# CAMMA-public/SelfPose3d

Hardware: AMD Instinct MI355X
Metric: multi-view samples/sec (5-view Panoptic, 80x80x20 voxel) (higher is better)
Workload: dtype f32

## Files before the change

### selfpose3d_amd/csrc/sp3d_winograd.hip

```cpp
#include <hip/hip_runtime.h>
#include <stdint.h>

#include "../../include/sp3d.h"

namespace sp3d {

__device__ __forceinline__ void bt4(float &d0, float &d1, float &d2, float &d3)
{
    const float t0 = d0 - d2, t1 = d1 + d2, t2 = d2 - d1, t3 = d1 - d3;
    d0 = t0; d1 = t1; d2 = t2; d3 = t3;
}

__global__ __launch_bounds__(256) void wino_input_kernel(const float *__restrict__ x, float *__restrict__ V, int B, int X,
                                                        int Y, int Z, int C, int TX, int TY, int TZ)
{
    const int64_t T = (int64_t)B * TX * TY * TZ;
    const int64_t gid = (int64_t)blockIdx.x * 256 + threadIdx.x;
    if (gid >= T * C) return;
    const int c = (int)(gid % C);
    int64_t t = gid / C;
    const int tz = (int)(t % TZ); int64_t r = t / TZ;
    const int ty = (int)(r % TY); r /= TY;
    const int tx = (int)(r % TX);
    const int b = (int)(r / TX);
// ... 407 lines not shown
            (void)r;
            w.mh = u32x4{0x3f803f80u + (unsigned)jk, 0x3f803f80u, 0x3f803f80u + (unsigned)i, 0x3f803f80u};
            w.l = u32x2{0x3f803f80u, 0x3f803f80u};
#else
            w.mh = *reinterpret_cast<const u32x4_a8 *>(r);
            w.l = *reinterpret_cast<const u32x2_a8 *>(r + 4);
#endif
            return w;
        };
        auto step = [&](int jk, int jk_next, const WfB (&bcur)[2], WfB (&bnxt)[2]) {
            const int j = jk >> 2, k = jk & 3;
            const int ya = (j == 0) ? 0 : ((j == 2) ? 2 : 1), yb = (j == 3) ? 3 : ((j == 2) ? 1 : 2);
            const int za = (k == 0) ? 0 : ((k == 2) ? 2 : 1), zb = (k == 3) ? 3 : ((k == 2) ? 1 : 2);
            const float sy = (j == 1) ? 1.0f : -1.0f, sz = (k == 1) ? 1.0f : -1.0f;
            const float *r00 = rb + (za * WF_RY + ya) * WF_ROW, *r10 = rb + (za * WF_RY + yb) * WF_ROW;
            const float *r01 = rb + (zb * WF_RY + ya) * WF_ROW, *r11 = rb + (zb * WF_RY + yb) * WF_ROW;
            WfB blate[2];
            blate[0] = load_b(2, jk);
            blate[1] = load_b(3, jk);
            float g[4][4];
#pragma unroll
            for (int xi = 0; xi < 4; ++xi) {
#if SP3D_W16_ABLATE & 8
                const float f0 = __int_as_float(0x3f800000 + jk + xi), f1 = __int_as_float(0x3f900000 + lane);
                const float4 v00 = make_float4(f0, f1, f0, f1), v10 = make_float4(f1, f0, f1, f0), v01 = v00, v11 = v10;
                (void)r00; (void)r10; (void)r01; (void)r11;
#else
                const float4 v00 = *reinterpret_cast<const float4 *>(r00 + xi * WF_VS), v10 = *reinterpret_cast<const float4 *>(r10 + xi * WF_VS);
                const float4 v01 = *reinterpret_cast<const float4 *>(r01 + xi * WF_VS), v11 = *reinterpret_cast<const float4 *>(r11 + xi * WF_VS);
#endif
                g[xi][0] = fmaf(sz, fmaf(sy, v11.x, v01.x), fmaf(sy, v10.x, v00.x));
                g[xi][1] = fmaf(sz, fmaf(sy, v11.y, v01.y), fmaf(sy, v10.y, v00.y));
                g[xi][2] = fmaf(sz, fmaf(sy, v11.z, v01.z), fmaf(sy, v10.z, v00.z));
                g[xi][3] = fmaf(sz, fmaf(sy, v11.w, v01.w), fmaf(sy, v10.w, v00.w));
            }
            float cyz[4];
#pragma unroll
            for (int bc = 0; bc < 4; ++bc) {
                const int bb = bc >> 1, c2 = bc & 1;
                const float cy = bb == 0 ? (j < 3 ? 1.0f : 0.0f) : (j == 0 ? 0.0f : (j == 1 ? 1.0f : -1.0f));
                const float cz = c2 == 0 ? (k < 3 ? 1.0f : 0.0f) : (k == 0 ? 0.0f : (k == 1 ? 1.0f : -1.0f));
                cyz[bc] = cy * cz;
            }
            f32x16 M0, M1;
#pragma unroll
            for (int v = 0; v < 16; ++v) { M0[v] = 0.0f; M1[v] = 0.0f; }
#pragma unroll
            for (int i = 0; i < 4; ++i) {
                float av[4];
#pragma unroll
                for (int kk = 0; kk < 4; ++kk)
                    av[kk] = (i == 1) ? g[1][kk] + g[2][kk] : ((i == 3) ? g[3][kk] - g[1][kk] : g[wf_ta(i)][kk] - g[wf_tb(i)][kk]);
                const unsigned hi01 = pack_bf16(av[0], av[1]), hi23 = pack_bf16(av[2], av[3]);
#if SP3D_W16_ABLATE & 4
                const unsigned mid01 = hi01, mid23 = hi23, lo01 = hi01, lo23 = hi23;
#else
                const float r0 = av[0] - bf16_lo(hi01), r1 = av[1] - bf16_hi(hi01), r2 = av[2] - bf16_lo(hi23), r3 = av[3] - bf16_hi(hi23);
                const unsigned mid01 = pack_bf16(r0, r1), mid23 = pack_bf16(r2, r3);
                const unsigned lo01 = pack_bf16(r0 - bf16_lo(mid01), r1 - bf16_hi(mid01));
                const unsigned lo23 = pack_bf16(r2 - bf16_lo(mid23), r3 - bf16_hi(mid23));
#endif
                const u32x4 Qhh = {hi01, hi23, hi01, hi23}, Qmm = {mid01, mid23, mid01, mid23}, Qlh = {lo01, lo23, hi01, hi23};
                const WfB &w = (i < 2) ? bcur[i] : blate[i - 2];
                const u32x4 Bmh = w.mh;
                const u32x4 Bhl = {w.mh.z, w.mh.w, w.l.x, w.l.y};
#if SP3D_W16_ABLATE & 1
                {
                    const unsigned z = (Qhh.x ^ Bmh.x) + (Qmm.y ^ Bmh.z) + (Qlh.x ^ Bhl.w) + (Qlh.z ^ Bhl.y);
                    M0[0] += __uint_as_float(z & 0x3fffffffu);
                    M1[1] += __uint_as_float((z >> 1) & 0x3fffffffu);
                    if (i == 1) {
                        bnxt[0] = load_b(0, jk_next);
                        bnxt[1] = load_b(1, jk_next);
                    }
                    continue;
                }
#endif
                if (i < 3) {
                    M0 = mfma_bf16(Qhh, Bmh, M0);
                    M0 = mfma_bf16(Qmm, Bmh, M0);
                    M0 = mfma_bf16(Qlh, Bhl, M0);
                }
                if (i == 1 || i == 3) {
                    M1 = mfma_bf16(Qhh, Bmh, M1);
                    M1 = mfma_bf16(Qmm, Bmh, M1);
                    M1 = mfma_bf16(Qlh, Bhl, M1);
                }
                if (i == 2) {
                    const u32x4 nmh = Bmh ^ 0x80008000u, nhl = Bhl ^ 0x80008000u;
                    M1 = mfma_bf16(Qhh, nmh, M1);
                    M1 = mfma_bf16(Qmm, nmh, M1);
                    M1 = mfma_bf16(Qlh, nhl, M1);
                }
                if (i == 1) {
                    bnxt[0] = load_b(0, jk_next);
                    bnxt[1] = load_b(1, jk_next);
                }
            }
#pragma unroll
            for (int bc = 0; bc < 4; ++bc) {
                const float coef = cyz[bc];
                if (coef != 0.0f) {
                    f32x16 cv;
#pragma unroll
                    for (int v = 0; v < 16; ++v) cv[v] = coef;
                    acc[bc] = __builtin_elementwise_fma(M0, cv, acc[bc]);
                    acc[4 + bc] = __builtin_elementwise_fma(M1, cv, acc[4 + bc]);
                }
            }
        };
        WfB b0[2], b1[2];
        b0[0] = load_b(0, 0);
        b0[1] = load_b(1, 0);
#pragma unroll 1
        for (int jk = 0; jk < 16; jk += 2) {
            step(jk, jk + 1, b0, b1);
            step(jk + 1, (jk + 2) & 15, b1, b0);
        }
    }

    const float sh = shift[t];
    const int yl = oy0 + 2 * h;
    const int64_t obase = ((((int64_t)b * X + ox0) * Y + yl) * Z + oz0) * O + t;
#pragma unroll
    for (int a = 0; a < 8; ++a) {
        float rv[16];
        if (MODE >= 2) {
#pragma unroll
            for (int v = 0; v < 16; ++v) {
                const int dx = 2 * (v & 3) + (a >> 2), dy = 4 * ((v >> 2) & 1) + ((a >> 1) & 1), dz = 2 * (v >> 3) + (a & 1);
                const int xo = min(ox0 + dx, X - 1), yo = min(yl + dy, Y - 1), zo = min(oz0 + dz, Z - 1);
                rv[v] = res[((((int64_t)b * X + xo) * Y + yo) * Z + zo) * O + t];
            }
        }
#pragma unroll
        for (int v = 0; v < 16; ++v) {
            const int dx = 2 * (v & 3) + (a >> 2), dy = 4 * ((v >> 2) & 1) + ((a >> 1) & 1), dz = 2 * (v >> 3) + (a & 1);
            if (ox0 + dx < X && oz0 + dz < Z && yl + dy < Y) {
                const int64_t idx = obase + (((int64_t)dx * Y + dy) * Z + dz) * O;
                float val = acc[a][v] + sh;
                if (MODE == 2) val += rv[v];
                if (MODE >= 1) val = fmaxf(val, 0.0f);
                if (MODE == 3) val += rv[v];
                y[idx] = val;
            }
        }
    }
}

typedef float f32x4 __attribute__((ext_vector_type(4)));
constexpr int W16_RX = 10, W16_RY = 10, W16_RZ = 4, W16_VS = 16;
constexpr int W16_ROW = W16_RX * W16_VS + 4;
constexpr int W16_LDS = W16_RY * W16_RZ * W16_ROW;

__device__ __forceinline__ f32x4 mfma16_bf16(u32x4 a, u32x4 b, f32x4 c)
{
    return __builtin_amdgcn_mfma_f32_16x16x32_bf16(__builtin_bit_cast(bf16x8, a), __builtin_bit_cast(bf16x8, b), c, 0, 0, 0);
}

template <int C, int MODE, int NBW, int KS>
__global__ __launch_bounds__(64 * (4 / NBW) * KS) __attribute__((amdgpu_waves_per_eu(NBW <= 2 ? 2 : 1))) void wino_fused16_kernel(const float *__restrict__ x,
                                                                          const unsigned *__restrict__ U3,
                                                                          float *__restrict__ y, const float *__restrict__ shift,
                                                                          const float *__restrict__ res, int B, int X, int Y,
                                                                          int Z, int NBX, int NBY, int NBZ)
{
    constexpr int O = 64, NCH = C / 16, NOW = 4 / NBW, NTG = 64 * NOW;
    static_assert(NCH % KS == 0, "chunks must divide evenly over the channel groups");
    __shared__ __attribute__((aligned(16))) float lds[KS * W16_LDS];
    const int tid = threadIdx.x, lane = tid & 63, wave = tid >> 6;
    const int kg = wave / NOW, ow = wave % NOW, tg = tid - kg * NTG;
    float *region = lds + kg * W16_LDS;
    const int tl = lane & 15, q = lane >> 4;
    int bid = blockIdx.x;
    const int bz = bid % NBZ; bid /= NBZ;
    const int by = bid % NBY; bid /= NBY;
    const int bx = bid % NBX;
    const int b = bid / NBX;
    const int ttx = tl & 3, tty = tl >> 2;
    const int ox0 = bx * 8, oy0 = by * 8, oz0 = bz * 2;
    const float *rb = region + (2 * tty) * W16_ROW + (2 * ttx) * W16_VS + 4 * q;

    f32x4 acc[8][NBW];
#pragma unroll
    for (int a = 0; a < 8; ++a)
#pragma unroll
        for (int n = 0; n < NBW; ++n) acc[a][n] = f32x4{0.0f, 0.0f, 0.0f, 0.0f};
#ifdef SP3D_W16_SETPRIO
    __builtin_amdgcn_s_setprio(SP3D_W16_SETPRIO);
#endif

    constexpr int NV4 = W16_RX * W16_RY * W16_RZ * 4, PER = (NV4 + NTG - 1) / NTG;
    int goff[PER], loff[PER];
#pragma unroll
    for (int u = 0; u < PER; ++u) {
        const int idx = tg + u * NTG;
        const int v = idx >> 2, part = idx & 3;
        const int vx = v % W16_RX, vy = (v / W16_RX) % W16_RY, vz = v / (W16_RX * W16_RY);
        const int gx = ox0 - 1 + vx, gy = oy0 - 1 + vy, gz = oz0 - 1 + vz;
        const bool in = idx < NV4 && gx >= 0 && gx < X && gy >= 0 && gy < Y && gz >= 0 && gz < Z;
        goff[u] = in ? (int)(((((int64_t)gx) * Y + gy) * Z + gz) * C + part * 4) : -1;
        loff[u] = idx < NV4 ? (vz * W16_RY + vy) * W16_ROW + vx * W16_VS + part * 4 : -1;
    }
    const float *xb = x + (int64_t)b * X * Y * Z * C;
    float4 pre[PER];
    auto fetch = [&](int cc) {
#pragma unroll
        for (int u = 0; u < PER; ++u) {
            pre[u] = make_float4(0.0f, 0.0f, 0.0f, 0.0f);
            if (goff[u] >= 0) pre[u] = *reinterpret_cast<const float4 *>(xb + goff[u] + cc * 16);
        }
    };
    fetch(kg);
#pragma unroll 1
    for (int cc = kg; cc < NCH; cc += KS) {
        __syncthreads();
#pragma unroll
        for (int u = 0; u < PER; ++u)
            if (loff[u] >= 0) *reinterpret_cast<float4 *>(region + loff[u]) = pre[u];
        __syncthreads();
        if (cc + KS < NCH) fetch(cc + KS);
        const unsigned *ub = U3 + ((((int64_t)cc * 4 + q) * O) + ow * NBW * 16 + tl) * 6;
        auto load_b = [&](int i, int jk, int n) {
            const unsigned *r = ub + (int64_t)(i * 16 + jk) * NCH * 4 * O * 6 + n * 16 * 6;
            WfB w;
            w.mh = *reinterpret_cast<const u32x4_a8 *>(r);
            w.l = *reinterpret_cast<const u32x2_a8 *>(r + 4);
            return w;
        };
#pragma unroll 1
        for (int jk = 0; jk < 16; ++jk) {
            const int j = jk >> 2, k = jk & 3;
            WfB bw[NBW][4];
#pragma unroll
            for (int n = 0; n < NBW; ++n)
#pragma unroll
                for (int i = 0; i < 4; ++i) {
#if SP3D_W16_ABLATE & 2
                    bw[n][i].mh = u32x4{0x3f803f80u + (unsigned)(jk + n), 0x3f803f80u, 0x3f803f80u + (unsigned)i, 0x3f803f80u};
                    bw[n][i].l = u32x2{0x3f803f80u, 0x3f803f80u};
#else
                    bw[n][i] = load_b(i, jk, n);
#endif
                }
            const int ya = (j == 0) ? 0 : ((j == 2) ? 2 : 1), yb = (j == 3) ? 3 : ((j == 2) ? 1 : 2);
            const int za = (k == 0) ? 0 : ((k == 2) ? 2 : 1), zb = (k == 3) ? 3 : ((k == 2) ? 1 : 2);
            const float sy = (j == 1) ? 1.0f : -1.0f, sz = (k == 1) ? 1.0f : -1.0f;
            const float *r00 = rb + (za * W16_RY + ya) * W16_ROW, *r10 = rb + (za * W16_RY + yb) * W16_ROW;
            const float *r01 = rb + (zb * W16_RY + ya) * W16_ROW, *r11 = rb + (zb * W16_RY + yb) * W16_ROW;
            float g[4][4];
#pragma unroll
            for (int xi = 0; xi < 4; ++xi) {
#if SP3D_W16_ABLATE & 8
                const float f0 = __int_as_float(0x3f800000 + jk + xi), f1 = __int_as_float(0x3f900000 + lane);
                const float4 v00 = make_float4(f0, f1, f0, f1), v10 = make_float4(f1, f0, f1, f0), v01 = v00, v11 = v10;
                (void)r00; (void)r10; (void)r01; (void)r11;
#else
                const float4 v00 = *reinterpret_cast<const float4 *>(r00 + xi * W16_VS), v10 = *reinterpret_cast<const float4 *>(r10 + xi * W16_VS);
                const float4 v01 = *reinterpret_cast<const float4 *>(r01 + xi * W16_VS), v11 = *reinterpret_cast<const float4 *>(r11 + xi * W16_VS);
#endif
                g[xi][0] = fmaf(sz, fmaf(sy, v11.x, v01.x), fmaf(sy, v10.x, v00.x));
                g[xi][1] = fmaf(sz, fmaf(sy, v11.y, v01.y), fmaf(sy, v10.y, v00.y));
                g[xi][2] = fmaf(sz, fmaf(sy, v11.z, v01.z), fmaf(sy, v10.z, v00.z));
                g[xi][3] = fmaf(sz, fmaf(sy, v11.w, v01.w), fmaf(sy, v10.w, v00.w));
            }
            float cyz[4];
#pragma unroll
            for (int bc = 0; bc < 4; ++bc) {
                const int bb = bc >> 1, c2 = bc & 1;
                const float cy = bb == 0 ? (j < 3 ? 1.0f : 0.0f) : (j == 0 ? 0.0f : (j == 1 ? 1.0f : -1.0f));
                const float cz = c2 == 0 ? (k < 3 ? 1.0f : 0.0f) : (k == 0 ? 0.0f : (k == 1 ? 1.0f : -1.0f));
                cyz[bc] = cy * cz;
            }
            f32x4 M0[NBW], M1[NBW];
#pragma unroll
            for (int n = 0; n < NBW; ++n) { M0[n] = f32x4{0.0f, 0.0f, 0.0f, 0.0f}; M1[n] = f32x4{0.0f, 0.0f, 0.0f, 0.0f}; }
#pragma unroll
            for (int i = 0; i < 4; ++i) {
                float av[4];
#pragma unroll
                for (int kk = 0; kk < 4; ++kk)
                    av[kk] = (i == 1) ? g[1][kk] + g[2][kk] : ((i == 3) ? g[3][kk] - g[1][kk] : g[wf_ta(i)][kk] - g[wf_tb(i)][kk]);
                const unsigned hi01 = pack_bf16(av[0], av[1]), hi23 = pack_bf16(av[2], av[3]);
#if SP3D_W16_ABLATE & 4
                const unsigned mid01 = hi01, mid23 = hi23, lo01 = hi01, lo23 = hi23;
#else
                const float r0 = av[0] - bf16_lo(hi01), r1 = av[1] - bf16_hi(hi01), r2 = av[2] - bf16_lo(hi23), r3 = av[3] - bf16_hi(hi23);
                const unsigned mid01 = pack_bf16(r0, r1), mid23 = pack_bf16(r2, r3);
                const unsigned lo01 = pack_bf16(r0 - bf16_lo(mid01), r1 - bf16_hi(mid01));
                const unsigned lo23 = pack_bf16(r2 - bf16_lo(mid23), r3 - bf16_hi(mid23));
#endif
                const u32x4 Qhh = {hi01, hi23, hi01, hi23}, Qmm = {mid01, mid23, mid01, mid23}, Qlh = {lo01, lo23, hi01, hi23};
#pragma unroll
                for (int n = 0; n < NBW; ++n) {
                    const WfB &w = bw[n][i];
                    const u32x4 Bmh = w.mh;
                    const u32x4 Bhl = {w.mh.z, w.mh.w, w.l.x, w.l.y};
#if SP3D_W16_ABLATE & 1
                    {
                        const unsigned z = (Qhh.x ^ Bmh.x) + (Qmm.y ^ Bmh.z) + (Qlh.x ^ Bhl.w) + (Qlh.z ^ Bhl.y);
                        M0[n].x += __uint_as_float(z & 0x3fffffffu);
                        M1[n].y += __uint_as_float((z >> 1) & 0x3fffffffu);
                        continue;
                    }
#endif
                    if (i < 3) {
                        M0[n] = mfma16_bf16(Qhh, Bmh, M0[n]);
                        M0[n] = mfma16_bf16(Qmm, Bmh, M0[n]);
                        M0[n] = mfma16_bf16(Qlh, Bhl, M0[n]);
                    }
                    if (i == 1 || i == 3) {
                        M1[n] = mfma16_bf16(Qhh, Bmh, M1[n]);
                        M1[n] = mfma16_bf16(Qmm, Bmh, M1[n]);
                        M1[n] = mfma16_bf16(Qlh, Bhl, M1[n]);
                    }
                    if (i == 2) {
                        const u32x4 nmh = Bmh ^ 0x80008000u, nhl = Bhl ^ 0x80008000u;
                        M1[n] = mfma16_bf16(Qhh, nmh, M1[n]);
                        M1[n] = mfma16_bf16(Qmm, nmh, M1[n]);
                        M1[n] = mfma16_bf16(Qlh, nhl, M1[n]);
                    }
                }
            }
#pragma unroll
            for (int n = 0; n < NBW; ++n)
#pragma unroll
                for (int bc = 0; bc < 4; ++bc) {
#if defined(SP3D_NO_PK) || defined(SP3D_W16_SCALAR_ACC)
                    for (int e = 0; e < 4; ++e) {
                        acc[bc][n][e] = fmaf(M0[n][e], cyz[bc], acc[bc][n][e]);
                        acc[4 + bc][n][e] = fmaf(M1[n][e], cyz[bc], acc[4 + bc][n][e]);
                    }
#else
                    const f32x4 cv = {cyz[bc], cyz[bc], cyz[bc], cyz[bc]};
                    acc[bc][n] = __builtin_elementwise_fma(M0[n], cv, acc[bc][n]);
                    acc[4 + bc][n] = __builtin_elementwise_fma(M1[n], cv, acc[4 + bc][n]);
#endif
                }
        }
    }

    if (KS > 1) {
        __syncthreads();
        f32x4 *red = reinterpret_cast<f32x4 *>(lds);
        if (kg > 0) {
#pragma unroll
            for (int a = 0; a < 8; ++a)
#pragma unroll
                for (int n = 0; n < NBW; ++n) red[(((kg - 1) * NOW + ow) * 8 * NBW + a * NBW + n) * 64 + lane] = acc[a][n];
        }
        __syncthreads();
        if (kg > 0) return;
#pragma unroll
        for (int g2 = 1; g2 < KS; ++g2)
#pragma unroll
            for (int a = 0; a < 8; ++a)
#pragma unroll
                for (int n = 0; n < NBW; ++n) acc[a][n] += red[(((g2 - 1) * NOW + ow) * 8 * NBW + a * NBW + n) * 64 + lane];
    }

    if (ox0 + 8 <= X && oy0 + 8 <= Y && oz0 + 2 <= Z) {
#pragma unroll
        for (int n = 0; n < NBW; ++n) {
            const int o = (ow * NBW + n) * 16 + tl;
            const float sh = shift[o];
            const int64_t obase = ((((int64_t)b * X + ox0) * Y + oy0) * Z + oz0) * O + o;
            int off[4];
#pragma unroll
            for (int v = 0; v < 4; ++v) off[v] = ((2 * v * Y + 2 * q) * Z) * O;
            float rv[8][4];
            if (MODE >= 2) {
#pragma unroll
                for (int a = 0; a < 8; ++a)
#pragma unroll
                    for (int v = 0; v < 4; ++v)
                        rv[a][v] = res[obase + off[v] + (((a >> 2) * Y + ((a >> 1) & 1)) * Z + (a & 1)) * O];
            }
#pragma unroll
            for (int a = 0; a < 8; ++a)
#pragma unroll
                for (int v = 0; v < 4; ++v) {
                    float val = acc[a][n][v] + sh;
                    if (MODE == 2) val += rv[a][v];
                    if (MODE >= 1) val = fmaxf(val, 0.0f);
                    if (MODE == 3) val += rv[a][v];
                    y[obase + off[v] + (((a >> 2) * Y + ((a >> 1) & 1)) * Z + (a & 1)) * O] = val;
                }
        }
        return;
    }
#pragma unroll
    for (int n = 0; n < NBW; ++n) {
        const int o = (ow * NBW + n) * 16 + tl;
        const float sh = shift[o];
        float rv[8][4];
        if (MODE >= 2) {
#pragma unroll
            for (int a = 0; a < 8; ++a)
#pragma unroll
                for (int v = 0; v < 4; ++v) {
                    const int tile = 4 * q + v;
                    const int rx = tile & 3, ry = tile >> 2;
                    const int xo = min(ox0 + 2 * rx + (a >> 2), X - 1), yo = min(oy0 + 2 * ry + ((a >> 1) & 1), Y - 1);
                    const int zo = min(oz0 + (a & 1), Z - 1);
                    rv[a][v] = res[((((int64_t)b * X + xo) * Y + yo) * Z + zo) * O + o];
                }
        }
#pragma unroll
        for (int a = 0; a < 8; ++a) {
#pragma unroll
            for (int v = 0; v < 4; ++v) {
                const int tile = 4 * q + v;
                const int rx = tile & 3, ry = tile >> 2;
                const int xo = ox0 + 2 * rx + (a >> 2), yo = oy0 + 2 * ry + ((a >> 1) & 1), zo = oz0 + (a & 1);
                if (xo < X && yo < Y && zo < Z) {
                    const int64_t idx = ((((int64_t)b * X + xo) * Y + yo) * Z + zo) * O + o;
                    float val = acc[a][n][v] + sh;
                    if (MODE == 2) val += rv[a][v];
                    if (MODE >= 1) val = fmaxf(val, 0.0f);
                    if (MODE == 3) val += rv[a][v];
                    y[idx] = val;
                }
            }
        }
    }
}


constexpr int CD_BX = 16, CD_BY = 8, CD_BZ = 4;
constexpr int CD_RX = CD_BX + 2, CD_RY = CD_BY + 2, CD_RZ = CD_BZ + 2, CD_VOX = 8, CD_ROW = CD_RX * CD_VOX, CD_ZP = CD_RY * CD_ROW + 4;
constexpr int CD_PLANE = CD_RZ * CD_ZP;
constexpr int CD_BUF = 2 * CD_PLANE;
constexpr int CD_NV4 = CD_RX * CD_RY * CD_RZ * 2;
constexpr int CD_PROD = 4;
constexpr int CD_PER = (CD_NV4 + 64 * CD_PROD - 1) / (64 * CD_PROD);
constexpr int CD_BUFS = ((CD_BUF / 4 + 63) / 64) * 256;
#ifndef SP3D_WG_ABLATE
#define SP3D_WG_ABLATE 0
#endif
struct CdRec { u32x4 hl, hh, mm; };


#ifdef SP3D_CD_TIMELINE
__device__ unsigned long long *g_cd_tl = nullptr;
#define CD_STAMP(slot) do { __builtin_amdgcn_sched_barrier(0); if (g_cd_tl && blockIdx.x == 0 && lane == 0 && item < 64) { g_cd_tl[(wave * 64 + item) * 4 + (slot)] = __builtin_readcyclecounter(); \
     \
    if (wave == 0 && (slot) == 0 && item == 0) { g_cd_tl[(7 * 64 + 62) * 4 + 0] = wall_clock64(); g_cd_tl[(7 * 64 + 62) * 4 + 1] = __builtin_readcyclecounter(); } \
    if (wave == 0 && (slot) == 3) { g_cd_tl[(7 * 64 + 63) * 4 + 0] = wall_clock64(); g_cd_tl[(7 * 64 + 63) * 4 + 1] = __builtin_readcyclecounter(); } } __builtin_amdgcn_sched_barrier(0); } while (0)
#else
#define CD_STAMP(slot) do { (void)item; } while (0)
#endif

__device__ __forceinline__ void split3(const float4 a, u32x4 &q0, u32x4 &q1)
{
    const unsigned hi01 = pack_bf16(a.x, a.y), hi23 = pack_bf16(a.z, a.w);
    const float r0 = __builtin_amdgcn_fmed3f(a.x - bf16_lo(hi01), 0.0f, a.x - bf16_lo(hi01));
    const float r1 = __builtin_amdgcn_fmed3f(a.y - bf16_hi(hi01), 0.0f, a.y - bf16_hi(hi01));
    const float r2 = __builtin_amdgcn_fmed3f(a.z - bf16_lo(hi23), 0.0f, a.z - bf16_lo(hi23));
    const float r3 = __builtin_amdgcn_fmed3f(a.w - bf16_hi(hi23), 0.0f, a.w - bf16_hi(hi23));
    const unsigned mid01 = pack_bf16(r0, r1), mid23 = pack_bf16(r2, r3);
    const unsigned lo01 = pack_bf16(r0 - bf16_lo(mid01), r1 - bf16_hi(mid01));
    const unsigned lo23 = pack_bf16(r2 - bf16_lo(mid23), r3 - bf16_hi(mid23));
    q0 = u32x4{lo01, lo23, hi01, hi23};
    q1 = u32x4{hi01, hi23, mid01, mid23};
}

template <int C, int MODE>
__global__ __launch_bounds__(64 * (4 + CD_PROD)) __attribute__((amdgpu_waves_per_eu(2, 2)))
void conv3_split_kernel(const float *__restrict__ x, const unsigned *__restrict__ W3, float *__restrict__ y,
                        const float *__restrict__ shift, const float *__restrict__ res, int B, int X, int Y, int Z, int NBX,
                        int NBY, int NBZ, int nblocks)
{
    constexpr int O = 32, NCH = C / 8;
    extern __shared__ __attribute__((aligned(16))) unsigned cd_lds[];
    const int tid = threadIdx.x, lane = tid & 63, wave = tid >> 6, t = lane & 31, h = lane >> 5;
    const int my_blocks = ((int)blockIdx.x < nblocks) ? (nblocks - 1 - (int)blockIdx.x) / (int)gridDim.x + 1 : 0;
    const int n_items = my_blocks * NCH;
    auto decode = [&](int item, int &b, int &ox0, int &oy0, int &oz0) {
        int bid = (int)blockIdx.x + (item / NCH) * (int)gridDim.x;
        const int bz = bid % NBZ; bid /= NBZ;
        const int by = bid % NBY; bid /= NBY;
        const int bx = bid % NBX;
        b = bid / NBX;
        ox0 = bx * CD_BX; oy0 = by * CD_BY; oz0 = bz * CD_BZ;
    };

    if (wave >= 4) {
        const int pt = tid - 256;
        __builtin_amdgcn_s_setprio(2);
        float4 d[CD_PER];
        int lo_[CD_PER], rel[CD_PER], vxyz[CD_PER];
#pragma unroll
        for (int u = 0; u < CD_PER; ++u) {
            const int idx = pt + 64 * CD_PROD * u;
            const int v = idx >> 1, half = idx & 1;
            const int vx = v % CD_RX, vy = (v / CD_RX) % CD_RY, vz = v / (CD_RX * CD_RY);
            lo_[u] = idx < CD_NV4 ? half * CD_PLANE + vz * CD_ZP + vy * CD_ROW + vx * CD_VOX : -1;
            rel[u] = ((vx * Y + vy) * Z + vz) * C + half * 4;
            vxyz[u] = idx < CD_NV4 ? (vx | (vy << 8) | (vz << 16)) : 0x00ffffff;
        }
        auto issue = [&](int k) {
            int b, ox0, oy0, oz0;
            decode(k, b, ox0, oy0, oz0);
            const int64_t vox0 = (((int64_t)b * X + (ox0 - 1)) * Y + (oy0 - 1)) * Z + (oz0 - 1);
            const float *xb = x + vox0 * C + (k % NCH) * 8;
            const int xlo = 1 - ox0, xhi = X + 1 - ox0, ylo = 1 - oy0, yhi = Y + 1 - oy0, zlo = 1 - oz0, zhi = Z + 1 - oz0;
#pragma unroll
            for (int u = 0; u < CD_PER; ++u) {
                const int vx = vxyz[u] & 255, vy = (vxyz[u] >> 8) & 255, vz = vxyz[u] >> 16;
                const bool in = vx >= xlo && vx < xhi && vy >= ylo && vy < yhi && vz >= zlo && vz < zhi;
                d[u] = make_float4(0.0f, 0.0f, 0.0f, 0.0f);
// ... 82 lines not shown
            if (st + 1 < 9) load_a(st + 1, a1);
#pragma unroll
            for (int dx = 0; dx < 3; ++dx) {
#pragma unroll
                for (int i = 0; i < 4; ++i) acc[i] = mfma_bf16(a0.lh[i + dx], w0.d[dx].hl, acc[i]);
#pragma unroll
                for (int i = 0; i < 4; ++i) acc[i] = mfma_bf16(a0.hm[i + dx], w0.d[dx].hh, acc[i]);
#pragma unroll
                for (int i = 0; i < 4; ++i) acc[i] = mfma_bf16(a0.hm[i + dx], w0.d[dx].mm, acc[i]);
            }
#pragma unroll
            for (int r = 0; r < 12; ++r) {
                __builtin_amdgcn_sched_group_barrier(0x008, 1, 0);
                __builtin_amdgcn_sched_group_barrier(0x100, 1, 0);
            }
#pragma unroll
            for (int r = 0; r < 9; ++r) {
                __builtin_amdgcn_sched_group_barrier(0x008, 1, 0);
                __builtin_amdgcn_sched_group_barrier(0x020, 1, 0);
            }
            __builtin_amdgcn_sched_group_barrier(0x008, 15, 0);
            __builtin_amdgcn_sched_barrier(0);
            a0 = a1;
            w0 = w1;
        }
        CD_STAMP(1);
        if (cc == NCH - 1) {
            int b, ox0, oy0, oz0;
            decode(item, b, ox0, oy0, oz0);
            if (ox0 + CD_BX <= X && oy0 + CD_BY <= Y && oz0 + CD_BZ <= Z) {
                const float sh = shift[t];
                const int64_t obase = ((((int64_t)b * X + ox0 + 4 * wave) * Y + oy0 + 4 * h) * Z + oz0) * O + t;
#pragma unroll
                for (int i = 0; i < 4; ++i)
#pragma unroll
                    for (int v = 0; v < 16; ++v) {
                        const int64_t idx = obase + (((int64_t)i * Y + (v & 3)) * Z + (v >> 2)) * O;
                        float val = acc[i][v] + sh;
                        if (MODE == 2) val += res[idx];
                        if (MODE >= 1) val = fmaxf(val, 0.0f);
                        if (MODE == 3) val += res[idx];
#if SP3D_W16_ABLATE & 16
                        if (val == 123.456f)
#endif
                        y[idx] = val;
                    }
            } else {
            float *scr = reinterpret_cast<float *>(cd_lds + 2 * CD_BUFS) + wave * 1024;
            const int g = lane & 7;
            const float4 sh4 = *reinterpret_cast<const float4 *>(shift + 4 * g);
#pragma unroll
            for (int mb = 0; mb < 4; ++mb) {
#pragma unroll
                for (int v = 0; v < 16; ++v) scr[(8 * (v >> 2) + (v & 3) + 4 * h) * 32 + t] = acc[mb][v];
                __builtin_amdgcn_fence(__ATOMIC_RELEASE, "wavefront");
                __builtin_amdgcn_wave_barrier();
#pragma unroll
                for (int r = 0; r < 4; ++r) {
                    const int m = (lane >> 3) + 8 * r;
                    float4 a = *reinterpret_cast<const float4 *>(scr + m * 32 + 4 * g);
                    const int xo = ox0 + 4 * wave + mb, yo = oy0 + (m & 7), zo = oz0 + (m >> 3);
                    if (xo < X && yo < Y && zo < Z) {
                        const int64_t vox = (((int64_t)b * X + xo) * Y + yo) * Z + zo;
                        a.x += sh4.x; a.y += sh4.y; a.z += sh4.z; a.w += sh4.w;
                        float4 rr = make_float4(0.0f, 0.0f, 0.0f, 0.0f);
                        if (MODE >= 2) rr = *reinterpret_cast<const float4 *>(res + vox * O + 4 * g);
                        if (MODE == 2) { a.x += rr.x; a.y += rr.y; a.z += rr.z; a.w += rr.w; }
                        if (MODE >= 1) { a.x = fmaxf(a.x, 0.0f); a.y = fmaxf(a.y, 0.0f); a.z = fmaxf(a.z, 0.0f); a.w = fmaxf(a.w, 0.0f); }
                        if (MODE == 3) { a.x += rr.x; a.y += rr.y; a.z += rr.z; a.w += rr.w; }
#if SP3D_W16_ABLATE & 16
                        if (a.x == 123.456f)
#endif
                        *reinterpret_cast<float4 *>(y + vox * O + 4 * g) = a;
                    }
                }
                __builtin_amdgcn_fence(__ATOMIC_RELEASE, "wavefront");
                __builtin_amdgcn_wave_barrier();
            }
            }
        }
        CD_STAMP(2);
        __syncthreads();
        CD_STAMP(3);
    }
}


}

extern "C" int sp3d_wino_fused(const float *x, const float *U, float *y, const float *shift, const float *residual, int mode,
                               int B, int X, int Y, int Z, int C, int O, void *stream)
{
    using namespace sp3d;
    if (B <= 0 || X <= 0 || Y <= 0 || Z <= 0 || mode < 0 || mode > 3) return SP3D_EINVAL;
    if (!x || !U || !y || !shift || (mode >= 2 && !residual)) return SP3D_ENULL;
    if (O != 32 || (C != 16 && C != 32)) return SP3D_EUNSUPPORTED;
    const int NBX = (X + 7) / 8, NBY = (Y + 7) / 8, NBZ = (Z + 3) / 4;
    const int64_t blocks = (int64_t)B * NBX * NBY * NBZ;
    if (blocks > 0x7fffffff) return SP3D_ERANGE;
    const dim3 grid((unsigned)blocks), block(64);
    hipStream_t s = (hipStream_t)stream;
#define SP3D_WF(C_, M_) hipLaunchKernelGGL((wino_fused_kernel<C_, M_>), grid, block, 0, s, x, U, y, shift, residual, B, X, Y, Z, NBX, NBY, NBZ)
#define SP3D_WFM(C_) switch (mode) { case 0: SP3D_WF(C_, 0); break; case 1: SP3D_WF(C_, 1); break; case 2: SP3D_WF(C_, 2); break; default: SP3D_WF(C_, 3); }
    if (C == 16) { SP3D_WFM(16) } else { SP3D_WFM(32) }
#undef SP3D_WFM
#undef SP3D_WF
    const hipError_t e = hipGetLastError();
    return e == hipSuccess ? SP3D_OK : (int)e;
}

extern "C" int sp3d_debug_wino_fused_timeline(void *dev_buffer)
{
#ifdef SP3D_WF_TIMELINE
    unsigned long long *p = (unsigned long long *)dev_buffer;
    return (int)hipMemcpyToSymbol(HIP_SYMBOL(sp3d::g_wf_tl), &p, sizeof(p));
#else
    (void)dev_buffer;
    return SP3D_EUNSUPPORTED;
#endif
}

extern "C" int sp3d_wino_fused_split(const float *x, const void *U3, float *y, const float *shift, const float *residual, int mode,
                                     int B, int X, int Y, int Z, int C, int O, void *stream)
{
    using namespace sp3d;
    if (B <= 0 || X <= 0 || Y <= 0 || Z <= 0 || mode < 0 || mode > 3) return SP3D_EINVAL;
    if (!x || !U3 || !y || !shift || (mode >= 2 && !residual)) return SP3D_ENULL;
    if (O != 32 || (C != 16 && C != 32) || (reinterpret_cast<uintptr_t>(U3) & 7)) return SP3D_EUNSUPPORTED;
    const int NBX = (X + 7) / 8, NBY = (Y + 7) / 8, NBZ = (Z + 3) / 4;
    const int64_t blocks = (int64_t)B * NBX * NBY * NBZ;
    if (blocks > 0x7fffffff) return SP3D_ERANGE;
    const dim3 grid((unsigned)blocks), block(64);
    hipStream_t s = (hipStream_t)stream;
    const unsigned *u3 = reinterpret_cast<const unsigned *>(U3);
#define SP3D_WF(C_, M_) hipLaunchKernelGGL((wino_fused3_kernel<C_, M_>), grid, block, 0, s, x, u3, y, shift, residual, B, X, Y, Z, NBX, NBY, NBZ)
#define SP3D_WFM(C_) switch (mode) { case 0: SP3D_WF(C_, 0); break; case 1: SP3D_WF(C_, 1); break; case 2: SP3D_WF(C_, 2); break; default: SP3D_WF(C_, 3); }
    if (C == 16) { SP3D_WFM(16) } else { SP3D_WFM(32) }
#undef SP3D_WFM
#undef SP3D_WF
    const hipError_t e = hipGetLastError();
    return e == hipSuccess ? SP3D_OK : (int)e;
}

extern "C" int sp3d_wino_fused_split64(const float *x, const void *U3, float *y, const float *shift, const float *residual,
                                       int mode, int B, int X, int Y, int Z, int C, int O, void *stream)
{
    using namespace sp3d;
    if (B <= 0 || X <= 0 || Y <= 0 || Z <= 0 || mode < 0 || mode > 3) return SP3D_EINVAL;
    if (!x || !U3 || !y || !shift || (mode >= 2 && !residual)) return SP3D_ENULL;
    if (O != 64 || (C != 32 && C != 64) || (reinterpret_cast<uintptr_t>(U3) & 7)) return SP3D_EUNSUPPORTED;
    const int NBX = (X + 7) / 8, NBY = (Y + 7) / 8, NBZ = (Z + 1) / 2;
    const int64_t blocks = (int64_t)B * NBX * NBY * NBZ;
    if (blocks > 0x7fffffff) return SP3D_ERANGE;
    constexpr int nbw = 2, ks = 2;
    hipStream_t s = (hipStream_t)stream;
    const unsigned *u3 = reinterpret_cast<const unsigned *>(U3);
    const dim3 grid((unsigned)blocks), block(64 * (4 / nbw) * ks);
#define SP3D_WF(C_, M_) hipLaunchKernelGGL((wino_fused16_kernel<C_, M_, 2, 2>), grid, block, 0, s, x, u3, y, shift, residual, B, X, Y, Z, NBX, NBY, NBZ)
#define SP3D_WFM(C_) switch (mode) { case 0: SP3D_WF(C_, 0); break; case 1: SP3D_WF(C_, 1); break; case 2: SP3D_WF(C_, 2); break; default: SP3D_WF(C_, 3); }
    if (C == 32) { SP3D_WFM(32) } else { SP3D_WFM(64) }
#undef SP3D_WFM
#undef SP3D_WF
    const hipError_t e = hipGetLastError();
    return e == hipSuccess ? SP3D_OK : (int)e;
}

extern "C" int sp3d_conv3_split(const float *x, const void *W3, float *y, const float *shift, const float *residual, int mode,
                                int B, int X, int Y, int Z, int C, int O, void *stream)
{
    using namespace sp3d;
    if (B <= 0 || X <= 0 || Y <= 0 || Z <= 0 || mode < 0 || mode > 3) return SP3D_EINVAL;
    if (!x || !W3 || !y || !shift || (mode >= 2 && !residual)) return SP3D_ENULL;
    if (O != 32 || (C != 16 && C != 32) || (reinterpret_cast<uintptr_t>(W3) & 15)) return SP3D_EUNSUPPORTED;
    if (reinterpret_cast<uintptr_t>(y) & 15) return SP3D_EUNSUPPORTED;
    if ((int64_t)X * Y * Z * C * 2 > 0x7fffffff) return SP3D_ERANGE;
    const int NBX = (X + CD_BX - 1) / CD_BX, NBY = (Y + CD_BY - 1) / CD_BY, NBZ = (Z + CD_BZ - 1) / CD_BZ;
    const int64_t blocks = (int64_t)B * NBX * NBY * NBZ;
    if (blocks > 0x7fffffff) return SP3D_ERANGE;
    static int cu_count[64] = {0};
    int dev = 0, cus = 256;
    if (hipGetDevice(&dev) == hipSuccess && dev >= 0 && dev < 64) {
        if (cu_count[dev] == 0) {
            int n = 0;
            cu_count[dev] = (hipDeviceGetAttribute(&n, hipDeviceAttributeMultiprocessorCount, dev) == hipSuccess && n > 0) ? n : 256;
        }
        cus = cu_count[dev];
    }
    const int rounds = (int)((blocks + cus - 1) / cus);
    const int nwg = (int)((blocks + rounds - 1) / rounds);
    const dim3 grid((unsigned)nwg), block(64 * (4 + CD_PROD));
    const size_t lds = (size_t)2 * CD_BUFS * sizeof(unsigned) + 4 * 1024 * sizeof(float);
    hipStream_t s = (hipStream_t)stream;
    const unsigned *w3 = reinterpret_cast<const unsigned *>(W3);
    int cd_dev = 0;
    { const hipError_t ed = hipGetDevice(&cd_dev); if (ed != hipSuccess) return (int)ed; }
    if (cd_dev < 0 || cd_dev >= 64) cd_dev = 63;
#define SP3D_CD(C_, M_) { static bool attr_dev[64] = {}; bool &attr = attr_dev[cd_dev]; if (!attr || cd_dev == 63) { hipError_t ea = hipFuncSetAttribute(reinterpret_cast<const void *>(conv3_split_kernel<C_, M_>), hipFuncAttributeMaxDynamicSharedMemorySize, (int)lds); if (ea != hipSuccess) return (int)ea; attr = true; } \
    hipLaunchKernelGGL((conv3_split_kernel<C_, M_>), grid, block, lds, s, x, w3, y, shift, residual, B, X, Y, Z, NBX, NBY, NBZ, (int)blocks); }
#define SP3D_CDI(C_) switch (mode) { case 0: SP3D_CD(C_, 0); break; case 1: SP3D_CD(C_, 1); break; case 2: SP3D_CD(C_, 2); break; default: SP3D_CD(C_, 3); }
    if (C == 16) { SP3D_CDI(16) } else { SP3D_CDI(32) }
#undef SP3D_CDI
#undef SP3D_CD
    const hipError_t e = hipGetLastError();
    return e == hipSuccess ? SP3D_OK : (int)e;
}

extern "C" int sp3d_debug_conv3_timeline(void *dev_buffer)
{
#ifdef SP3D_CD_TIMELINE
    unsigned long long *p = (unsigned long long *)dev_buffer;
    return (int)hipMemcpyToSymbol(HIP_SYMBOL(sp3d::g_cd_tl), &p, sizeof(p));
#else
    (void)dev_buffer;
    return SP3D_EUNSUPPORTED;
#endif
}
```

Before: 2768.

## Replace split-K Winograd kernel with cooperative input-transform kernel sharing bf16 operands via LDS

The split64 fused Winograd kernel is replaced by a new kernel. Its four waves each compute the input transform for one j slice and write the three-way bf16-split operands into shared memory. All waves then read those operands for MFMA, instead of every wave recomputing the transform for all 16 (j,k) pairs. Work is split over j halves plus output halves, with a single reduction at the end. Weight loads are software-pipelined one step ahead, and per-thread offset arrays are recomputed inline to save registers. The change adds two barriers per k step and extra LDS traffic for the operands. It also references a split3 helper that is only forward-declared here.

```diff
diff --git a/selfpose3d_amd/csrc/sp3d_winograd.hip b/selfpose3d_amd/csrc/sp3d_winograd.hip
--- a/selfpose3d_amd/csrc/sp3d_winograd.hip
+++ b/selfpose3d_amd/csrc/sp3d_winograd.hip
@@ -583,26 +583,29 @@
 constexpr int W16_RX = 10, W16_RY = 10, W16_RZ = 4, W16_VS = 16;
 constexpr int W16_ROW = W16_RX * W16_VS + 4;
 constexpr int W16_LDS = W16_RY * W16_RZ * W16_ROW;
+constexpr int W16_QP = 64 * 4;
+constexpr int W16_OPS = 16 * 2 * W16_QP;
 
 __device__ __forceinline__ f32x4 mfma16_bf16(u32x4 a, u32x4 b, f32x4 c)
 {
     return __builtin_amdgcn_mfma_f32_16x16x32_bf16(__builtin_bit_cast(bf16x8, a), __builtin_bit_cast(bf16x8, b), c, 0, 0, 0);
 }
 
-template <int C, int MODE, int NBW, int KS>
-__global__ __launch_bounds__(64 * (4 / NBW) * KS) __attribute__((amdgpu_waves_per_eu(NBW <= 2 ? 2 : 1))) void wino_fused16_kernel(const float *__restrict__ x,
-                                                                          const unsigned *__restrict__ U3,
-                                                                          float *__restrict__ y, const float *__restrict__ shift,
-                                                                          const float *__restrict__ res, int B, int X, int Y,
-                                                                          int Z, int NBX, int NBY, int NBZ)
-{
-    constexpr int O = 64, NCH = C / 16, NOW = 4 / NBW, NTG = 64 * NOW;
-    static_assert(NCH % KS == 0, "chunks must divide evenly over the channel groups");
-    __shared__ __attribute__((aligned(16))) float lds[KS * W16_LDS];
-    const int tid = threadIdx.x, lane = tid & 63, wave = tid >> 6;
-    const int kg = wave / NOW, ow = wave % NOW, tg = tid - kg * NTG;
-    float *region = lds + kg * W16_LDS;
-    const int tl = lane & 15, q = lane >> 4;
+__device__ __forceinline__ void split3(const float4 a, u32x4 &q0, u32x4 &q1);
+
+template <int C, int MODE>
+__global__ __launch_bounds__(256) __attribute__((amdgpu_waves_per_eu(2, 2)))
+void wino_half_kernel(const float *__restrict__ x, const unsigned *__restrict__ U3, float *__restrict__ y,
+                      const float *__restrict__ shift, const float *__restrict__ res, int B, int X, int Y, int Z, int NBX,
+                      int NBY, int NBZ)
+{
+    constexpr int O = 64, NCH = C / 16, NBW = 2, NT = 256;
+    __shared__ __attribute__((aligned(16))) float region[W16_LDS];
+    __shared__ __attribute__((aligned(16))) unsigned ops[W16_OPS];
+    const int tid = threadIdx.x;
+    int lane = tid & 63, wave = __builtin_amdgcn_readfirstlane(tid >> 6);
+    int ow = wave & 1, jh = wave >> 1;
+    int tl = lane & 15, q = lane >> 4;
     int bid = blockIdx.x;
     const int bz = bid % NBZ; bid /= NBZ;
     const int by = bid % NBY; bid /= NBY;
@@ -617,177 +620,182 @@
     for (int a = 0; a < 8; ++a)
 #pragma unroll
         for (int n = 0; n < NBW; ++n) acc[a][n] = f32x4{0.0f, 0.0f, 0.0f, 0.0f};
-#ifdef SP3D_W16_SETPRIO
-    __builtin_amdgcn_s_setprio(SP3D_W16_SETPRIO);
-#endif
-
-    constexpr int NV4 = W16_RX * W16_RY * W16_RZ * 4, PER = (NV4 + NTG - 1) / NTG;
-    int goff[PER], loff[PER];
-#pragma unroll
-    for (int u = 0; u < PER; ++u) {
-        const int idx = tg + u * NTG;
-        const int v = idx >> 2, part = idx & 3;
-        const int vx = v % W16_RX, vy = (v / W16_RX) % W16_RY, vz = v / (W16_RX * W16_RY);
-        const int gx = ox0 - 1 + vx, gy = oy0 - 1 + vy, gz = oz0 - 1 + vz;
-        const bool in = idx < NV4 && gx >= 0 && gx < X && gy >= 0 && gy < Y && gz >= 0 && gz < Z;
-        goff[u] = in ? (int)(((((int64_t)gx) * Y + gy) * Z + gz) * C + part * 4) : -1;
-        loff[u] = idx < NV4 ? (vz * W16_RY + vy) * W16_ROW + vx * W16_VS + part * 4 : -1;
-    }
+
+    constexpr int NV4 = W16_RX * W16_RY * W16_RZ * 4, PER = (NV4 + NT - 1) / NT;
     const float *xb = x + (int64_t)b * X * Y * Z * C;
     float4 pre[PER];
     auto fetch = [&](int cc) {
 #pragma unroll
         for (int u = 0; u < PER; ++u) {
+            int idx = tid + u * NT;
+            asm volatile("" : "+v"(idx));
+            const int v = idx >> 2, part = idx & 3;
+            const int vx = v % W16_RX, vy = (v / W16_RX) % W16_RY, vz = v / (W16_RX * W16_RY);
+            const int gx = ox0 - 1 + vx, gy = oy0 - 1 + vy, gz = oz0 - 1 + vz;
+            const bool in = idx < NV4 && gx >= 0 && gx < X && gy >= 0 && gy < Y && gz >= 0 && gz < Z;
             pre[u] = make_float4(0.0f, 0.0f, 0.0f, 0.0f);
-            if (goff[u] >= 0) pre[u] = *reinterpret_cast<const float4 *>(xb + goff[u] + cc * 16);
+            if (in) pre[u] = *reinterpret_cast<const float4 *>(xb + ((((int64_t)gx) * Y + gy) * Z + gz) * C + part * 4 + cc * 16);
         }
     };
-    fetch(kg);
+    auto stage = [&]() {
+#pragma unroll
+        for (int u = 0; u < PER; ++u) {
+            int idx = tid + u * NT;
+            asm volatile("" : "+v"(idx));
+            const int v = idx >> 2, part = idx & 3;
+            const int vx = v % W16_RX, vy = (v / W16_RX) % W16_RY, vz = v / (W16_RX * W16_RY);
+            if (idx < NV4) *reinterpret_cast<float4 *>(region + (vz * W16_RY + vy) * W16_ROW + vx * W16_VS + part * 4) = pre[u];
+        }
+    };
+
+    const unsigned lane_w = (unsigned)((q * O + ow * NBW * 16 + tl) * 6);
+    struct WRec { u32x2 m; u32x4 hl; };
+    struct WStep { WRec w[NBW][4]; };
+    auto load_w = [&](WStep &ws, int i, int cc, int j, int k) {
+        unsigned lw = lane_w;
+        asm volatile("" : "+v"(lw));
+#pragma unroll
+        for (int n = 0; n < NBW; ++n) {
+            const unsigned *r = U3 + (((int64_t)(i * 16 + j * 4 + k) * NCH + cc) * 4 * O + n * 16) * 6 + lw;
+            ws.w[n][i].m = *reinterpret_cast<const u32x2_a8 *>(r);
+            ws.w[n][i].hl = *reinterpret_cast<const u32x4_a8 *>(r + 2);
+        }
+    };
+    unsigned *op = ops + lane * 4;
+
+    auto step = [&](WStep &ws, int j, int k, int jn, int kn, int cn) {
+        u32x4 qa[4][2];
+#pragma unroll
+        for (int i = 0; i < 4; ++i) {
+            qa[i][0] = *reinterpret_cast<const u32x4 *>(op + ((i * 4 + j) * 2 + 0) * W16_QP);
+            qa[i][1] = *reinterpret_cast<const u32x4 *>(op + ((i * 4 + j) * 2 + 1) * W16_QP);
+        }
+        float cyz[4];
+#pragma unroll
+        for (int bc = 0; bc < 4; ++bc) {
+            const int bb = bc >> 1, c2 = bc & 1;
+            const float cy = bb == 0 ? (j < 3 ? 1.0f : 0.0f) : (j == 0 ? 0.0f : (j == 1 ? 1.0f : -1.0f));
+            const float cz = c2 == 0 ? (k < 3 ? 1.0f : 0.0f) : (k == 0 ? 0.0f : (k == 1 ? 1.0f : -1.0f));
+            cyz[bc] = cy * cz;
+        }
+        f32x4 M0[NBW], M1[NBW];
+#pragma unroll
+        for (int n = 0; n < NBW; ++n) { M0[n] = f32x4{0.0f, 0.0f, 0.0f, 0.0f}; M1[n] = f32x4{0.0f, 0.0f, 0.0f, 0.0f}; }
+#pragma unroll
+        for (int i = 0; i < 4; ++i) {
+            const u32x4 Qlh = qa[i][0], Qhm = qa[i][1];
+            const u32x4 nlh = Qlh ^ 0x80008000u, nhm = Qhm ^ 0x80008000u;
+#pragma unroll
+            for (int n = 0; n < NBW; ++n) {
+                const WRec &w = ws.w[n][i];
+                const u32x4 Bhh = {w.hl.x, w.hl.y, w.hl.x, w.hl.y}, Bmm = {w.m.x, w.m.y, w.m.x, w.m.y};
+                const u32x4 Bhl = w.hl;
+                if (i < 3) {
+                    M0[n] = mfma16_bf16(Qhm, Bhh, M0[n]);
+                    M0[n] = mfma16_bf16(Qhm, Bmm, M0[n]);
+                    M0[n] = mfma16_bf16(Qlh, Bhl, M0[n]);
+                }
+                if (i == 1 || i == 3) {
+                    M1[n] = mfma16_bf16(Qhm, Bhh, M1[n]);
+                    M1[n] = mfma16_bf16(Qhm, Bmm, M1[n]);
+                    M1[n] = mfma16_bf16(Qlh, Bhl, M1[n]);
+                }
+                if (i == 2) {
+                    M1[n] = mfma16_bf16(nhm, Bhh, M1[n]);
+                    M1[n] = mfma16_bf16(nhm, Bmm, M1[n]);
+                    M1[n] = mfma16_bf16(nlh, Bhl, M1[n]);
+                }
+            }
+            load_w(ws, i, cn, jn, kn);
+        }
+#pragma unroll
+        for (int n = 0; n < NBW; ++n)
+#pragma unroll
+            for (int bc = 0; bc < 4; ++bc) {
+#if defined(SP3D_NO_PK)
+                for (int e = 0; e < 4; ++e) {
+                    acc[bc][n][e] = fmaf(M0[n][e], cyz[bc], acc[bc][n][e]);
+                    acc[4 + bc][n][e] = fmaf(M1[n][e], cyz[bc], acc[4 + bc][n][e]);
+                }
+#else
+                const f32x4 cv = {cyz[bc], cyz[bc], cyz[bc], cyz[bc]};
+                acc[bc][n] = __builtin_elementwise_fma(M0[n], cv, acc[bc][n]);
+                acc[4 + bc][n] = __builtin_elementwise_fma(M1[n], cv, acc[4 + bc][n]);
+#endif
+            }
+    };
+
+    fetch(0);
+    WStep ws;
+#pragma unroll
+    for (int i = 0; i < 4; ++i) load_w(ws, i, 0, 2 * jh, 0);
+    stage();
 #pragma unroll 1
-    for (int cc = kg; cc < NCH; cc += KS) {
+    for (int cc = 0; cc < NCH; ++cc) {
+#pragma unroll 1
+        for (int k = 0; k < 4; ++k) {
+            const bool refill = k == 3 && cc + 1 < NCH;
+            __syncthreads();
+            if (refill) fetch(cc + 1);
+            {
+                const int j = wave;
+                const int ya = (j == 0) ? 0 : ((j == 2) ? 2 : 1), yb = (j == 3) ? 3 : ((j == 2) ? 1 : 2);
+                const int za = (k == 0) ? 0 : ((k == 2) ? 2 : 1), zb = (k == 3) ? 3 : ((k == 2) ? 1 : 2);
+                const float sy = (j == 1) ? 1.0f : -1.0f, sz = (k == 1) ? 1.0f : -1.0f;
+                const float *r00 = rb + (za * W16_RY + ya) * W16_ROW, *r10 = rb + (za * W16_RY + yb) * W16_ROW;
+                const float *r01 = rb + (zb * W16_RY + ya) * W16_ROW, *r11 = rb + (zb * W16_RY + yb) * W16_ROW;
+                float g[4][4];
+#pragma unroll
+                for (int xi = 0; xi < 4; ++xi) {
+                    const float4 v00 = *reinterpret_cast<const float4 *>(r00 + xi * W16_VS), v10 = *reinterpret_cast<const float4 *>(r10 + xi * W16_VS);
+                    const float4 v01 = *reinterpret_cast<const float4 *>(r01 + xi * W16_VS), v11 = *reinterpret_cast<const float4 *>(r11 + xi * W16_VS);
+                    g[xi][0] = fmaf(sz, fmaf(sy, v11.x, v01.x), fmaf(sy, v10.x, v00.x));
+                    g[xi][1] = fmaf(sz, fmaf(sy, v11.y, v01.y), fmaf(sy, v10.y, v00.y));
+                    g[xi][2] = fmaf(sz, fmaf(sy, v11.z, v01.z), fmaf(sy, v10.z, v00.z));
+                    g[xi][3] = fmaf(sz, fmaf(sy, v11.w, v01.w), fmaf(sy, v10.w, v00.w));
+                }
+#pragma unroll
+                for (int i = 0; i < 4; ++i) {
+                    float av[4];
+#pragma unroll
+                    for (int kk = 0; kk < 4; ++kk)
+                        av[kk] = (i == 1) ? g[1][kk] + g[2][kk] : ((i == 3) ? g[3][kk] - g[1][kk] : g[wf_ta(i)][kk] - g[wf_tb(i)][kk]);
+                    u32x4 q0, q1;
+                    split3(make_float4(av[0], av[1], av[2], av[3]), q0, q1);
+                    *reinterpret_cast<u32x4 *>(op + ((i * 4 + j) * 2 + 0) * W16_QP) = q0;
+                    *reinterpret_cast<u32x4 *>(op + ((i * 4 + j) * 2 + 1) * W16_QP) = q1;
+                }
+            }
+            __syncthreads();
+            if (refill) stage();
+            const int kn = (k + 1) & 3, cn = (k == 3) ? ((cc + 1 < NCH) ? cc + 1 : 0) : cc;
+            step(ws, 2 * jh, k, 2 * jh + 1, k, cc);
+            step(ws, 2 * jh + 1, k, 2 * jh, kn, cn);
+        }
+    }
+
+    {
+        int t2 = threadIdx.x;
+        asm volatile("" : "+v"(t2));
+        lane = t2 & 63; wave = __builtin_amdgcn_readfirstlane(t2 >> 6);
+        ow = wave & 1; jh = wave >> 1;
+        tl = lane & 15; q = lane >> 4;
+    }
+    __syncthreads();
+    {
+        f32x4 *red = reinterpret_cast<f32x4 *>(ops);
+        if (jh > 0) {
+#pragma unroll
+            for (int a = 0; a < 8; ++a)
+#pragma unroll
+                for (int n = 0; n < NBW; ++n) red[((ow * 8 + a) * NBW + n) * 64 + lane] = acc[a][n];
+        }
         __syncthreads();
-#pragma unroll
-        for (int u = 0; u < PER; ++u)
-            if (loff[u] >= 0) *reinterpret_cast<float4 *>(region + loff[u]) = pre[u];
-        __syncthreads();
-        if (cc + KS < NCH) fetch(cc + KS);
-        const unsigned *ub = U3 + ((((int64_t)cc * 4 + q) * O) + ow * NBW * 16 + tl) * 6;
-        auto load_b = [&](int i, int jk, int n) {
-            const unsigned *r = ub + (int64_t)(i * 16 + jk) * NCH * 4 * O * 6 + n * 16 * 6;
-            WfB w;
-            w.mh = *reinterpret_cast<const u32x4_a8 *>(r);
-            w.l = *reinterpret_cast<const u32x2_a8 *>(r + 4);
-            return w;
-        };
-#pragma unroll 1
-        for (int jk = 0; jk < 16; ++jk) {
-            const int j = jk >> 2, k = jk & 3;
-            WfB bw[NBW][4];
-#pragma unroll
-            for (int n = 0; n < NBW; ++n)
-#pragma unroll
-                for (int i = 0; i < 4; ++i) {
-#if SP3D_W16_ABLATE & 2
-                    bw[n][i].mh = u32x4{0x3f803f80u + (unsigned)(jk + n), 0x3f803f80u, 0x3f803f80u + (unsigned)i, 0x3f803f80u};
-                    bw[n][i].l = u32x2{0x3f803f80u, 0x3f803f80u};
-#else
-                    bw[n][i] = load_b(i, jk, n);
-#endif
-                }
-            const int ya = (j == 0) ? 0 : ((j == 2) ? 2 : 1), yb = (j == 3) ? 3 : ((j == 2) ? 1 : 2);
-            const int za = (k == 0) ? 0 : ((k == 2) ? 2 : 1), zb = (k == 3) ? 3 : ((k == 2) ? 1 : 2);
-            const float sy = (j == 1) ? 1.0f : -1.0f, sz = (k == 1) ? 1.0f : -1.0f;
-            const float *r00 = rb + (za * W16_RY + ya) * W16_ROW, *r10 = rb + (za * W16_RY + yb) * W16_ROW;
-            const float *r01 = rb + (zb * W16_RY + ya) * W16_ROW, *r11 = rb + (zb * W16_RY + yb) * W16_ROW;
-            float g[4][4];
-#pragma unroll
-            for (int xi = 0; xi < 4; ++xi) {
-#if SP3D_W16_ABLATE & 8
-                const float f0 = __int_as_float(0x3f800000 + jk + xi), f1 = __int_as_float(0x3f900000 + lane);
-                const float4 v00 = make_float4(f0, f1, f0, f1), v10 = make_float4(f1, f0, f1, f0), v01 = v00, v11 = v10;
-                (void)r00; (void)r10; (void)r01; (void)r11;
-#else
-                const float4 v00 = *reinterpret_cast<const float4 *>(r00 + xi * W16_VS), v10 = *reinterpret_cast<const float4 *>(r10 + xi * W16_VS);
-                const float4 v01 = *reinterpret_cast<const float4 *>(r01 + xi * W16_VS), v11 = *reinterpret_cast<const float4 *>(r11 + xi * W16_VS);
-#endif
-                g[xi][0] = fmaf(sz, fmaf(sy, v11.x, v01.x), fmaf(sy, v10.x, v00.x));
-                g[xi][1] = fmaf(sz, fmaf(sy, v11.y, v01.y), fmaf(sy, v10.y, v00.y));
-                g[xi][2] = fmaf(sz, fmaf(sy, v11.z, v01.z), fmaf(sy, v10.z, v00.z));
-                g[xi][3] = fmaf(sz, fmaf(sy, v11.w, v01.w), fmaf(sy, v10.w, v00.w));
-            }
-            float cyz[4];
-#pragma unroll
-            for (int bc = 0; bc < 4; ++bc) {
-                const int bb = bc >> 1, c2 = bc & 1;
-                const float cy = bb == 0 ? (j < 3 ? 1.0f : 0.0f) : (j == 0 ? 0.0f : (j == 1 ? 1.0f : -1.0f));
-                const float cz = c2 == 0 ? (k < 3 ? 1.0f : 0.0f) : (k == 0 ? 0.0f : (k == 1 ? 1.0f : -1.0f));
-                cyz[bc] = cy * cz;
-            }
-            f32x4 M0[NBW], M1[NBW];
-#pragma unroll
-            for (int n = 0; n < NBW; ++n) { M0[n] = f32x4{0.0f, 0.0f, 0.0f, 0.0f}; M1[n] = f32x4{0.0f, 0.0f, 0.0f, 0.0f}; }
-#pragma unroll
-            for (int i = 0; i < 4; ++i) {
-                float av[4];
-#pragma unroll
-                for (int kk = 0; kk < 4; ++kk)
-                    av[kk] = (i == 1) ? g[1][kk] + g[2][kk] : ((i == 3) ? g[3][kk] - g[1][kk] : g[wf_ta(i)][kk] - g[wf_tb(i)][kk]);
-                const unsigned hi01 = pack_bf16(av[0], av[1]), hi23 = pack_bf16(av[2], av[3]);
-#if SP3D_W16_ABLATE & 4
-                const unsigned mid01 = hi01, mid23 = hi23, lo01 = hi01, lo23 = hi23;
-#else
-                const float r0 = av[0] - bf16_lo(hi01), r1 = av[1] - bf16_hi(hi01), r2 = av[2] - bf16_lo(hi23), r3 = av[3] - bf16_hi(hi23);
-                const unsigned mid01 = pack_bf16(r0, r1), mid23 = pack_bf16(r2, r3);
-                const unsigned lo01 = pack_bf16(r0 - bf16_lo(mid01), r1 - bf16_hi(mid01));
-                const unsigned lo23 = pack_bf16(r2 - bf16_lo(mid23), r3 - bf16_hi(mid23));
-#endif
-                const u32x4 Qhh = {hi01, hi23, hi01, hi23}, Qmm = {mid01, mid23, mid01, mid23}, Qlh = {lo01, lo23, hi01, hi23};
-#pragma unroll
-                for (int n = 0; n < NBW; ++n) {
-                    const WfB &w = bw[n][i];
-                    const u32x4 Bmh = w.mh;
-                    const u32x4 Bhl = {w.mh.z, w.mh.w, w.l.x, w.l.y};
-#if SP3D_W16_ABLATE & 1
-                    {
-                        const unsigned z = (Qhh.x ^ Bmh.x) + (Qmm.y ^ Bmh.z) + (Qlh.x ^ Bhl.w) + (Qlh.z ^ Bhl.y);
-                        M0[n].x += __uint_as_float(z & 0x3fffffffu);
-                        M1[n].y += __uint_as_float((z >> 1) & 0x3fffffffu);
-                        continue;
-                    }
-#endif
-                    if (i < 3) {
-                        M0[n] = mfma16_bf16(Qhh, Bmh, M0[n]);
-                        M0[n] = mfma16_bf16(Qmm, Bmh, M0[n]);
-                        M0[n] = mfma16_bf16(Qlh, Bhl, M0[n]);
-                    }
-                    if (i == 1 || i == 3) {
-                        M1[n] = mfma16_bf16(Qhh, Bmh, M1[n]);
-                        M1[n] = mfma16_bf16(Qmm, Bmh, M1[n]);
-                        M1[n] = mfma16_bf16(Qlh, Bhl, M1[n]);
-                    }
-                    if (i == 2) {
-                        const u32x4 nmh = Bmh ^ 0x80008000u, nhl = Bhl ^ 0x80008000u;
-                        M1[n] = mfma16_bf16(Qhh, nmh, M1[n]);
-                        M1[n] = mfma16_bf16(Qmm, nmh, M1[n]);
-                        M1[n] = mfma16_bf16(Qlh, nhl, M1[n]);
-                    }
-                }
-            }
-#pragma unroll
-            for (int n = 0; n < NBW; ++n)
-#pragma unroll
-                for (int bc = 0; bc < 4; ++bc) {
-#if defined(SP3D_NO_PK) || defined(SP3D_W16_SCALAR_ACC)
-                    for (int e = 0; e < 4; ++e) {
-                        acc[bc][n][e] = fmaf(M0[n][e], cyz[bc], acc[bc][n][e]);
-                        acc[4 + bc][n][e] = fmaf(M1[n][e], cyz[bc], acc[4 + bc][n][e]);
-                    }
-#else
-                    const f32x4 cv = {cyz[bc], cyz[bc], cyz[bc], cyz[bc]};
-                    acc[bc][n] = __builtin_elementwise_fma(M0[n], cv, acc[bc][n]);
-                    acc[4 + bc][n] = __builtin_elementwise_fma(M1[n], cv, acc[4 + bc][n]);
-#endif
-                }
-        }
-    }
-
-    if (KS > 1) {
-        __syncthreads();
-        f32x4 *red = reinterpret_cast<f32x4 *>(lds);
-        if (kg > 0) {
-#pragma unroll
-            for (int a = 0; a < 8; ++a)
-#pragma unroll
-                for (int n = 0; n < NBW; ++n) red[(((kg - 1) * NOW + ow) * 8 * NBW + a * NBW + n) * 64 + lane] = acc[a][n];
-        }
-        __syncthreads();
-        if (kg > 0) return;
-#pragma unroll
-        for (int g2 = 1; g2 < KS; ++g2)
-#pragma unroll
-            for (int a = 0; a < 8; ++a)
-#pragma unroll
-                for (int n = 0; n < NBW; ++n) acc[a][n] += red[(((g2 - 1) * NOW + ow) * 8 * NBW + a * NBW + n) * 64 + lane];
+        if (jh > 0) return;
+#pragma unroll
+        for (int a = 0; a < 8; ++a)
+#pragma unroll
+            for (int n = 0; n < NBW; ++n) acc[a][n] += red[((ow * 8 + a) * NBW + n) * 64 + lane];
     }
 
     if (ox0 + 8 <= X && oy0 + 8 <= Y && oz0 + 2 <= Z) {
@@ -1176,11 +1184,10 @@
     const int NBX = (X + 7) / 8, NBY = (Y + 7) / 8, NBZ = (Z + 1) / 2;
     const int64_t blocks = (int64_t)B * NBX * NBY * NBZ;
     if (blocks > 0x7fffffff) return SP3D_ERANGE;
-    constexpr int nbw = 2, ks = 2;
     hipStream_t s = (hipStream_t)stream;
     const unsigned *u3 = reinterpret_cast<const unsigned *>(U3);
-    const dim3 grid((unsigned)blocks), block(64 * (4 / nbw) * ks);
-#define SP3D_WF(C_, M_) hipLaunchKernelGGL((wino_fused16_kernel<C_, M_, 2, 2>), grid, block, 0, s, x, u3, y, shift, residual, B, X, Y, Z, NBX, NBY, NBZ)
+    const dim3 grid((unsigned)blocks), block(256);
+#define SP3D_WF(C_, M_) hipLaunchKernelGGL((wino_half_kernel<C_, M_>), grid, block, 0, s, x, u3, y, shift, residual, B, X, Y, Z, NBX, NBY, NBZ)
 #define SP3D_WFM(C_) switch (mode) { case 0: SP3D_WF(C_, 0); break; case 1: SP3D_WF(C_, 1); break; case 2: SP3D_WF(C_, 2); break; default: SP3D_WF(C_, 3); }
     if (C == 32) { SP3D_WFM(32) } else { SP3D_WFM(64) }
 #undef SP3D_WFM
```

Result: slower. 2704 (-2.3%).
